# baoxuezhao/GPU-mapreduce

Measured on AMD Instinct MI355X. Metric: KV-pairs/sec (whole node), InvertedIndex end-to-end, higher is better.
Workload: dtype bytes+int32 (no float compute in MapReduce); 1 GPU; model=InvertedIndex, global_batch=1073741824, seq_len=134217728, parallelism=dp1, bytes_per_gpu=1073741824, link_gap=200

## Files before the change

### csrc/engine/engine.cpp

```cpp
#include "hostarena.h"
#include "kv.h"
#include "xfer.h"
#include "grouper.h"

#include <ATen/hip/HIPContext.h>
#include <algorithm>
#include <chrono>
#include <cstring>
#include <condition_variable>
#include <cstdlib>
#include <map>
#include <mutex>
#include <thread>
#include <numeric>
#include <stdexcept>

#include "../kernels/hashfn.h"
#include "../kernels/launch.h"
#include "../kernels/rmatfn.h"

namespace mrh {

namespace {

// ... 1596 lines not shown
  at::Tensor out = at::empty({nval}, opt(dev, at::kLong));
  const int64_t* sp = P0<int64_t>(seg);
  int64_t* o = P0<int64_t>(out);
  int64_t s = 0;
  for (int64_t i = 0; i < nval; ++i) {
    while (s + 1 < nseg && sp[s + 1] <= i) ++s;
    o[i] = s;
  }
  return out;
}

at::Tensor bincount_dev(const at::Tensor& idx_in, int64_t K) {
  const at::Device dev = idx_in.device();
  at::Tensor idx = idx_in.to(at::kLong).contiguous();
  at::Tensor c = at::zeros({std::max<int64_t>(K, 0)}, opt(dev, at::kLong));
  if (idx.numel() == 0 || K <= 0) return c;
  if (dev.is_cuda()) {
    k::histogram(P0<int64_t>(idx), idx.numel(), K, P0<int64_t>(c), cur_stream());
    return c;
  }
  const int64_t* p = P0<int64_t>(idx);
  int64_t* o = P0<int64_t>(c);
  for (int64_t i = 0; i < idx.numel(); ++i)
    if (p[i] >= 0 && p[i] < K) o[p[i]]++;
  return c;
}

at::Tensor mask_indices(const at::Tensor& mask_in) {
  const at::Device dev = mask_in.device();
  at::Tensor m = mask_in.to(at::kBool).contiguous().view(at::kByte);
  const int64_t n = m.numel();
  if (!dev.is_cuda()) return at::nonzero(m).view({-1});
  if (n == 0) return at::empty({0}, opt(dev, at::kLong));
  at::Tensor f = at::empty({n}, opt(dev, at::kLong));
  k::mask_flags(P0<uint8_t>(m), n, P0<int64_t>(f), cur_stream());
  at::Tensor pos = exclusive_scan(f);
  const int64_t cnt = pos[n].item<int64_t>();
  at::Tensor out = at::empty({cnt}, opt(dev, at::kLong));
  if (cnt) k::compact_mask(P0<uint8_t>(m), P0<int64_t>(pos), n, P0<int64_t>(out), cur_stream());
  return out;
}

at::Tensor repeat_index(const at::Tensor& counts) {
  at::Tensor off = exclusive_scan(counts.to(at::kLong));
  const int64_t n = counts.numel();
  const int64_t tot = n ? off[n].item<int64_t>() : 0;
  return segment_ids(off, n, tot);
}

KV expand(const KMV& kmv) {
  at::Tensor sid = segment_ids(kmv.seg, kmv.nkey, kmv.nval);
  KV out;
  out.n = kmv.nval;
  out.kw = kmv.keys.kw;
  out.kdata = gather_rows(kmv.keys.kdata, kmv.keys.koff, kmv.keys.kw, sid, &out.koff);
  out.vw = kmv.vw;
  out.vdata = kmv.vdata;
  out.voff = kmv.voff;
  return out;
}

KMV sort_multivalues(const KMV& kmv, int flag) {
  if (kmv.nval <= 1) return kmv;
  const at::Device dev = kmv.seg.device();
  at::Tensor perm1 = sort_perm_column(kmv.vdata, kmv.voff, kmv.vw, kmv.nval, flag);
  at::Tensor sid = segment_ids(kmv.seg, kmv.nkey, kmv.nval);
  at::Tensor sid_p = sid.index_select(0, perm1.to(at::kLong));
  auto [ks, perm2, passes] = radix_sort_pairs(sid_p, iota_u32(kmv.nval, dev), 0, 64);
  at::Tensor perm = perm1.to(at::kLong).index_select(0, perm2.to(at::kLong));
  KMV out = kmv;
  out.vdata = gather_rows(kmv.vdata, kmv.voff, kmv.vw, perm, &out.voff);
  return out;
}


KV map_urls(const at::Tensor& text, int64_t n, int32_t doc_id) {
  const at::Device dev = text.device();
  if (text.numel() < n + 32) fail("map_urls: text buffer must be padded by >= 32 bytes");
  KV kv;
  kv.kw = -1;
  kv.vw = 4;
  if (dev.is_cuda()) {
    auto s = cur_stream();
    int64_t nt = k::url_num_tiles(n);
    at::Tensor cnt = at::empty({std::max<int64_t>(nt, 1)}, opt(dev, at::kInt));
    k::url_count(P0<uint8_t>(text), n, P0<uint32_t>(cnt), s);
    at::Tensor toff = scan_u32(cnt.narrow(0, 0, nt));
    int64_t nurl = (int64_t)(uint32_t)toff[nt].item<int32_t>();
    at::Tensor starts = at::empty({std::max<int64_t>(nurl, 1)}, opt(dev, at::kLong));
    k::url_emit_starts(P0<uint8_t>(text), n, P0<uint32_t>(toff), P0<int64_t>(starts), s);
    at::Tensor klen = at::empty({std::max<int64_t>(nurl, 1)}, opt(dev, at::kInt));
    k::url_lengths(P0<uint8_t>(text), n, P0<int64_t>(starts), nurl, P0<int32_t>(klen), s);
    kv.koff = exclusive_scan(klen.narrow(0, 0, nurl));
    int64_t kb = scalar_i64(kv.koff, nurl);
    kv.kdata = at::empty({kb}, opt(dev, at::kByte));
    k::url_copy(P0<uint8_t>(text), P0<int64_t>(starts), P0<int64_t>(kv.koff), nurl, P0<uint8_t>(kv.kdata), s);
    at::Tensor v = at::empty({nurl}, opt(dev, at::kInt));
    k::fill_i32(P0<int32_t>(v), nurl, doc_id, s);
    kv.vdata = v.view(at::kByte);
    kv.n = nurl;
    return kv;
  }
  const uint8_t* t = P0<uint8_t>(text);
  static const char pat[] = "<a href=\"";
  std::vector<int64_t> koff{0};
  std::vector<uint8_t> kd;
  for (int64_t i = 0; i + 8 < n; ++i) {
    if (memcmp(t + i, pat, 9) != 0) continue;
    int64_t a = i + 9, j = a;
    while (j < n && t[j] != '"') ++j;
    kd.insert(kd.end(), t + a, t + j);
    kd.push_back(0);
    koff.push_back((int64_t)kd.size());
  }
  kv.n = (int64_t)koff.size() - 1;
  kv.koff = at::from_blob(koff.data(), {(int64_t)koff.size()}, opt(at::kCPU, at::kLong)).clone();
  kv.kdata = at::from_blob(kd.data(), {(int64_t)kd.size()}, opt(at::kCPU, at::kByte)).clone();
  kv.vdata = at::full({kv.n}, doc_id, opt(at::kCPU, at::kInt)).view(at::kByte);
  return kv;
}

static inline bool is_ws(uint8_t c) { return c == ' ' || c == '\t' || c == '\n' || c == '\f' || c == '\r' || c == 0; }

KV map_words(const at::Tensor& text, int64_t n) {
  const at::Device dev = text.device();
  if (text.numel() < n + 32) fail("map_words: text buffer must be padded by >= 32 bytes");
  KV kv;
  kv.kw = -1;
  kv.vw = 0;
  kv.vdata = at::empty({0}, opt(dev, at::kByte));
  if (dev.is_cuda()) {
    auto s = cur_stream();
    const int64_t nt = k::tok_num_tiles(n);
    if (nt <= 0) {
      kv.n = 0;
      kv.koff = at::zeros({1}, opt(dev, at::kLong));
      kv.kdata = at::empty({0}, opt(dev, at::kByte));
      return kv;
    }
    at::Tensor cw = at::empty({nt}, opt(dev, at::kInt)), cb = at::empty({nt}, opt(dev, at::kInt));
    k::tok_count2(P0<uint8_t>(text), n, P0<uint32_t>(cw), P0<uint32_t>(cb), s);
    at::Tensor tw = scan_u32(cw);
    at::Tensor tb = exclusive_scan(cb);
    uint32_t nw32 = 0;
    int64_t kb = 0;
    read_small(s, {{P0<uint32_t>(tw) + nt, &nw32, 4}, {P0<int64_t>(tb) + nt, &kb, 8}});
    const int64_t nw = (int64_t)nw32;
    kv.koff = at::empty({nw + 1}, opt(dev, at::kLong));
    kv.kdata = at::empty({kb}, opt(dev, at::kByte));
    k::tok_emit2(P0<uint8_t>(text), n, P0<uint32_t>(tw), P0<int64_t>(tb), P0<int64_t>(kv.koff), P0<uint8_t>(kv.kdata),
                 s);
    k::fill_i64(P0<int64_t>(kv.koff) + nw, 1, kb, s);
    kv.n = nw;
    return kv;
  }
  const uint8_t* t = P0<uint8_t>(text);
  std::vector<int64_t> koff{0};
  std::vector<uint8_t> kd;
  for (int64_t i = 0; i < n;) {
    while (i < n && is_ws(t[i])) ++i;
    if (i >= n) break;
    int64_t j = i;
    while (j < n && !is_ws(t[j])) ++j;
    kd.insert(kd.end(), t + i, t + j);
    kd.push_back(0);
    koff.push_back((int64_t)kd.size());
    i = j;
  }
  kv.n = (int64_t)koff.size() - 1;
  kv.koff = at::from_blob(koff.data(), {(int64_t)koff.size()}, opt(at::kCPU, at::kLong)).clone();
  kv.kdata = at::from_blob(kd.data(), {(int64_t)kd.size()}, opt(at::kCPU, at::kByte)).clone();
  return kv;
}

KV map_rmat(int64_t nedges, int nlevels, double a, double b, double c, double d, double fraction, uint64_t seed,
            uint64_t first_edge, at::Device dev) {
  KV kv;
  kv.kw = 16;
  kv.vw = 0;
  kv.n = nedges;
  kv.vdata = at::empty({0}, opt(dev, at::kByte));
// ... 16 lines not shown
```

### csrc/kernels/group.hip

```cpp
#include <algorithm>

#include "common.h"
#include "launch.h"

namespace mrh {
namespace k {
namespace {

using dev::rot32;

constexpr int NT = 256;
constexpr int32_t NONE = -1;

unsigned blocks_for(int64_t n) {
  int64_t b = (n + NT - 1) / NT;
  return (unsigned)(b < 1 ? 1 : (b > (1 << 20) ? (1 << 20) : b));
}

__device__ __forceinline__ uint64_t nz(uint64_t h) { return h ? h : 1ull; }
__device__ __forceinline__ uint64_t home(uint64_t h, uint64_t mask) { return (h ^ (h >> 32)) & mask; }

struct Keys {
  const uint8_t* d;
  const int64_t* off;
  int w;
  __device__ __forceinline__ const uint8_t* at(int64_t r) const { return off ? d + off[r] : d + r * (int64_t)w; }
  __device__ __forceinline__ int64_t len(int64_t r) const { return off ? off[r + 1] - off[r] : (int64_t)w; }
};

__device__ __forceinline__ void load_key16(const uint8_t* p, int64_t len, uint32_t w[4]) {
  const uintptr_t a = reinterpret_cast<uintptr_t>(p);
  const uint32_t* q = reinterpret_cast<const uint32_t*>(a & ~uintptr_t(3));
  const uint32_t r = (uint32_t)(a & 3);
  const int nb = len < 16 ? (int)len : 16;
  const int nd = (int)((r + nb + 3) >> 2);
  uint32_t d[5];
#pragma unroll
  for (int j = 0; j < 5; ++j) d[j] = j < nd ? q[j] : 0u;
#pragma unroll
  for (int j = 0; j < 4; ++j) {
    uint32_t v = r ? __builtin_amdgcn_alignbyte(d[j + 1], d[j], r) : d[j];
    const int valid = nb - 4 * j;
    if (valid <= 0) v = 0;
    else if (valid < 4) v &= (1u << (8 * valid)) - 1u;
    w[j] = v;
  }
}

__device__ __forceinline__ uint64_t hash64_words(const uint32_t w[4], int64_t len) {
  uint32_t a, b, c;
  a = b = c = 0xdeadbeefu + (uint32_t)len + 0x9e3779b9u;
  c += 0x7f4a7c15u;
  if (len == 0) return ((uint64_t)c << 32) | b;
  a += w[0];
  b += w[1];
  c += w[2];
  if (len > 12) {
    MRH_L3_MIX(a, b, c);
    a += w[3];
  }
  MRH_L3_FINAL(a, b, c);
  return ((uint64_t)c << 32) | b;
}

__device__ __forceinline__ uint64_t ld_l2_u64(const void* p) {
  return __hip_atomic_load(reinterpret_cast<const unsigned long long*>(p), __ATOMIC_RELAXED,
                           __HIP_MEMORY_SCOPE_AGENT);
}

__global__ __launch_bounds__(NT) void k_dict_insert(Keys K, const uint64_t* __restrict__ h, int64_t n, int64_t row0,
                                                   DictTable T, int32_t* __restrict__ gid, int retry) {
  unsigned long long bad = 0, left = 0;
  const int64_t stride = (int64_t)gridDim.x * NT;
  for (int64_t i = (int64_t)blockIdx.x * NT + threadIdx.x; i - threadIdx.x < n; i += stride) {
    const int64_t row = row0 + i;
    bool live = i < n;
    if (live && retry) live = gid[row] == NONE;
    unsigned long long hv = 0;
    const uint8_t* p = nullptr;
    int64_t len = 0;
    uint32_t w[4] = {0, 0, 0, 0};
    uint64_t s = 0;
    uint4 hdr = make_uint4(0, 0, 0, 0);
    int state = 0;
    if (live) {
      p = K.at(row);
      len = K.len(row);
      load_key16(p, len, w);
      if (h) {
        hv = nz(h[i]);
      } else if (len <= 16) {
        hv = nz(hash64_words(w, len));
      } else {
        uint32_t c = 0x9e3779b9u, b = 0x7f4a7c15u;
        dev::lookup3_wide(p, len, &c, &b);
        hv = nz(((uint64_t)c << 32) | b);
      }
      s = home(hv, T.mask);
      for (uint64_t probe = 0;; ++probe) {
        hdr = *reinterpret_cast<const uint4*>(&T.slots[s]);
        unsigned long long v = ((unsigned long long)hdr.y << 32) | hdr.x;
        if (v == 0) {
          if (__hip_atomic_load(&T.ctr[3], __ATOMIC_RELAXED, __HIP_MEMORY_SCOPE_AGENT)) {
            state = 3;
            break;
          }
          v = atomicCAS(&T.slots[s].hash, 0ull, hv);
          if (v == 0) {
            state = 2;
            break;
          }
          hdr.z = 0;
        }
        if (v == hv) {
          state = 1;
          break;
        }
        s = (s + 1) & T.mask;
        if (probe >= T.mask) {
          state = 3;
          break;
        }
      }
    }
    int32_t g = NONE;
    if (state == 2) {
      g = (int32_t)atomicAdd(&T.ctr[0], 1ull);
      DictSlot& sl = T.slots[s];
      sl.len = (int32_t)len;
      *reinterpret_cast<uint4*>(sl.key) = make_uint4(w[0], w[1], w[2], w[3]);
      T.rep[g] = row;
      T.ghash[g] = hv;
      __hip_atomic_store(&sl.gid1, g + 1, __ATOMIC_RELEASE, __HIP_MEMORY_SCOPE_AGENT);
      if ((int64_t)g + 1 >= T.limit) __hip_atomic_store(&T.ctr[3], 1ull, __ATOMIC_RELAXED, __HIP_MEMORY_SCOPE_AGENT);
    }
    if (state == 1) {
      const DictSlot& sl = T.slots[s];
      bool fresh = false;
      while (hdr.z == 0) {
        __builtin_amdgcn_s_sleep(1);
        const uint64_t gl = ld_l2_u64(&sl.gid1);
        hdr.z = (uint32_t)gl;
        hdr.w = (uint32_t)(gl >> 32);
        fresh = true;
      }
      g = (int32_t)hdr.z - 1;
      uint4 kk = fresh ? make_uint4(0, 0, 0, 0) : *reinterpret_cast<const uint4*>(sl.key);
      bool same = !fresh && (int64_t)(int32_t)hdr.w == len && kk.x == w[0] && kk.y == w[1] && kk.z == w[2] &&
                  kk.w == w[3];
      if (!same) {
        const uint64_t k01 = ld_l2_u64(&sl.key[0]), k23 = ld_l2_u64(&sl.key[2]);
        const uint64_t gl = ld_l2_u64(&sl.gid1);
        same = (int64_t)(int32_t)(gl >> 32) == len && (uint32_t)k01 == w[0] && (uint32_t)(k01 >> 32) == w[1] &&
               (uint32_t)k23 == w[2] && (uint32_t)(k23 >> 32) == w[3];
      }
      if (same && len > 16) {
        int64_t b = T.rep[g];
        if (b < 0) b = (int64_t)ld_l2_u64(&T.rep[g]);
        same = dev::bytes_equal(p + 16, K.at(b) + 16, len - 16);
      }
      if (!same) ++bad;
    }
    if (state == 3) ++left;
    if (live) gid[row] = g;
  }
  bad = dev::wave_sum(bad);
  left = dev::wave_sum(left);
  if (dev::lane_id() == 0) {
    if (bad) atomicAdd(&T.ctr[1], bad);
    if (left) atomicAdd(&T.ctr[2], left);
  }
}

constexpr int HW = 32768;
constexpr int HNT = 1024;
constexpr int kDictHistRows = 256;

__global__ __launch_bounds__(HNT) void k_dict_hist(const int32_t* __restrict__ gid, int64_t n, int64_t w0,
                                                  int64_t wlen, uint32_t* __restrict__ partial) {
  __shared__ uint32_t hist[HW];
  for (int j = threadIdx.x; j < HW; j += HNT) hist[j] = 0;
  __syncthreads();
  const int64_t n4 = n >> 2;
  const int4* g4 = reinterpret_cast<const int4*>(gid);
  auto add = [&](int32_t g) {
    const uint64_t d = (uint64_t)((int64_t)g - w0);
// ... 178 lines not shown
```

### csrc/kernels/launch.h

```cpp
#pragma once
#include <hip/hip_runtime.h>
#include <cstddef>
#include <cstdint>

namespace mrh {
namespace k {

size_t scan_temp_bytes(int64_t n);
void exclusive_scan_u32(const uint32_t* in, uint32_t* out, int64_t n, void* temp, hipStream_t s);
void exclusive_scan_i64(const int64_t* in, int64_t* out, int64_t n, void* temp, hipStream_t s);
void lengths_to_offsets(const int32_t* len, int64_t* off, int64_t n, void* temp, hipStream_t s);

size_t radix_temp_bytes(int64_t n);
void radix_sort_u64_u32(const uint64_t* keys_in, const uint32_t* vals_in, uint64_t* keys_out,
                        uint32_t* vals_out, uint64_t* keys_alt, uint32_t* vals_alt, int64_t n,
                        int begin_bit, int end_bit, void* temp, hipStream_t s,
                        int* passes_run = nullptr, bool skip_trivial = true);

void hash32_fixed(const uint8_t* kdata, int kw, int64_t n, uint32_t seed, uint32_t* out, hipStream_t s);
void hash32_var(const uint8_t* kdata, const int64_t* koff, int64_t n, uint32_t seed, uint32_t* out,
                hipStream_t s);
void hash64_fixed(const uint8_t* kdata, int kw, int64_t n, uint64_t* out, hipStream_t s);
void hash64_var(const uint8_t* kdata, const int64_t* koff, int64_t n, uint64_t* out, hipStream_t s);
void partition_dest(const uint32_t* h, int64_t n, int P, int32_t* dest, int64_t* counts, hipStream_t s);

int part_tile();
void part_count(const int32_t* dest_in, const uint8_t* kd, int kw, const int64_t* koff, const int64_t* voff,
                int64_t n, int P, int nb, int32_t* dest_out, int64_t* cnt, int64_t* kbytes, int64_t* vbytes,
                hipStream_t s);
void part_scatter(const int32_t* dest, int64_t n, int P, int nb, const int64_t* cbase, const uint8_t* kd, int kw,
                  const uint8_t* vd, int vw, const int64_t* koff, const int64_t* voff, uint8_t* ksend,
                  uint8_t* vsend, int64_t* perm, int32_t* klen, int32_t* vlen, hipStream_t s);
void copy_var_i64(const uint8_t* src, const int64_t* soff, const int64_t* perm, int64_t n, uint8_t* dst,
                  const int64_t* doff, hipStream_t s);
void part_header(const int64_t* cs, const int64_t* ks, const int64_t* vs, int P, int nb, int kw, int vw,
                 int64_t kcode, int64_t vcode, int64_t* hdr, hipStream_t s);
void count_mod(const int64_t* v, int64_t n, int P, int64_t* counts, hipStream_t s);
void piece_bytes(const int64_t* soff, const int64_t* start, int P, int R, int64_t* out, hipStream_t s);

void seg_marks(const int64_t* seg, int64_t nseg, int64_t nval, int64_t* marks, hipStream_t s);
void histogram(const int64_t* idx, int64_t n, int64_t K, int64_t* counts, hipStream_t s);
void nz_flags(const uint64_t* v, int64_t n, int32_t* f, hipStream_t s);
void compact_nz(const uint64_t* v, const int64_t* pos, int64_t n, int64_t* out, hipStream_t s);
void mask_flags(const uint8_t* m, int64_t n, int64_t* f, hipStream_t s);
void compact_mask(const uint8_t* m, const int64_t* pos, int64_t n, int64_t* out, hipStream_t s);
void lookup_sorted(const int64_t* keys, int64_t n, const int64_t* q, int64_t m, int64_t* idx, hipStream_t s);

void make_sortkeys_fixed(const uint8_t* data, int w, int64_t n, int mode, bool descending,
                         uint64_t* keys, uint32_t* idx, hipStream_t s);
void make_sortkeys_strprefix(const uint8_t* data, const int64_t* off, int64_t n, int64_t start,
                             bool descending, uint64_t* keys, uint32_t* idx, hipStream_t s);
void iota_u32(uint32_t* idx, int64_t n, hipStream_t s);
void str_groups(const uint64_t* ks, const uint8_t* alive, const uint32_t* head_in, int64_t n, bool desc,
                uint32_t* head_out, hipStream_t s);
void str_active(const uint64_t* ks, const uint8_t* alive, const uint32_t* head, int64_t n, bool desc, uint32_t* active,
                hipStream_t s);
void str_refine(const uint32_t* active, const uint32_t* pos, const uint32_t* gid_incl, const uint32_t* perm,
                const uint8_t* data, const int64_t* off, int64_t n, int64_t start, bool desc, int32_t* where,
                uint64_t* nk, uint64_t* gk, hipStream_t s);
void str_apply(const uint32_t* order, const int32_t* where, const uint64_t* nk, int64_t m, const uint32_t* perm_in,
               uint32_t* perm_out, uint64_t* ks, uint8_t* alive, hipStream_t s);
void gather_fixed(const uint8_t* src, int w, const uint32_t* idx, int64_t n, uint8_t* dst, hipStream_t s);
void gather_fixed_i64idx(const uint8_t* src, int w, const int64_t* idx, int64_t n, uint8_t* dst,
                         hipStream_t s);
void gather_var_lengths(const int64_t* src_off, const uint32_t* idx, int64_t n, int32_t* len,
                        hipStream_t s);
void gather_var_copy(const uint8_t* src, const int64_t* src_off, const uint32_t* idx, int64_t n,
                     uint8_t* dst, const int64_t* dst_off, hipStream_t s);
void head_flags_u64(const uint64_t* keys, int64_t n, uint32_t* flags, hipStream_t s);
void compact_heads(const uint32_t* flags, const uint32_t* pos, int64_t n, int64_t* seg, hipStream_t s);
struct PackShifts {
  int nw;
  int s[8];
};
void pack_words(const uint64_t* kd, int64_t n, const PackShifts& sh, uint64_t* out, uint32_t* idx, hipStream_t s);
void pack_kv(const uint64_t* kd, const uint64_t* vd, int64_t n, const PackShifts& sh, uint64_t* out, hipStream_t s);
void pack_kv_split(const uint64_t* kd, const void* vd, int vw, int64_t n, const PackShifts& sh, int vbits, int B, int hi,
                   uint64_t* out, int32_t* bkt, hipStream_t s);
void unpack_split(const uint64_t* heads, int64_t m, int bucket, int B, int hi, const PackShifts& sh,
                  const PackShifts& bits, uint64_t* keys, hipStream_t s);
void split_values(const uint64_t* words, int64_t n, int vbits, int vw, void* vout, hipStream_t s);
int64_t seg_packed_tiles(int64_t n);
void seg_packed_count(const uint64_t* w, int64_t n, int vb, uint64_t km, int64_t* tcnt, hipStream_t s);
void seg_packed_write(const uint64_t* w, int64_t n, int vb, uint64_t km, const int64_t* tbase, int64_t* seg,
                      uint64_t* heads, void* vout, int vw, hipStream_t s);
void bits_count(const uint64_t* H, int64_t nw, uint32_t* cnt, hipStream_t s);
void bits_compact(const uint64_t* H, int64_t nw, const uint32_t* pos, int64_t n, int64_t* seg, hipStream_t s);
void verify_groups_var(const uint8_t* kdata, const int64_t* koff, const uint32_t* perm,
                       const uint32_t* flags, const uint32_t* pos, const int64_t* seg, int64_t n,
                       unsigned long long* mismatches, hipStream_t s);
void verify_groups_fixed(const uint8_t* kdata, int kw, const uint32_t* perm, const uint32_t* flags,
                         const uint32_t* pos, const int64_t* seg, int64_t n,
                         unsigned long long* mismatches, hipStream_t s);
void dest_byte_counts(const int32_t* dest, const int64_t* off, int64_t n, int P, int64_t* bytes,
                      hipStream_t s);
void offsets_to_lengths(const int64_t* off, int64_t n, int32_t* len, hipStream_t s);

void seg_reduce(const void* vals, int dtype, int op, const int64_t* seg, int64_t nseg, int64_t nval, void* out,
                hipStream_t s);
void seg_count(const int64_t* seg, int64_t nseg, int32_t* out, hipStream_t s);

int64_t url_num_tiles(int64_t n);
void url_count(const uint8_t* text, int64_t n, uint32_t* tile_counts, hipStream_t s);
void url_emit_starts(const uint8_t* text, int64_t n, const uint32_t* tile_off, int64_t* starts,
                     hipStream_t s);
void url_lengths(const uint8_t* text, int64_t n, const int64_t* starts, int64_t nurl,
                 int32_t* keylen, hipStream_t s);
void url_copy(const uint8_t* text, const int64_t* starts, const int64_t* koff, int64_t nurl,
              uint8_t* kdata, hipStream_t s);
int64_t tok_num_tiles(int64_t n);
void tok_count2(const uint8_t* text, int64_t n, uint32_t* tile_words, uint32_t* tile_bytes, hipStream_t s);
void tok_emit2(const uint8_t* text, int64_t n, const uint32_t* toff_w, const int64_t* toff_b, int64_t* koff,
               uint8_t* kd, hipStream_t s);
void tok_count(const uint8_t* text, int64_t n, uint32_t* tile_counts, hipStream_t s);
void tok_emit(const uint8_t* text, int64_t n, const uint32_t* tile_off, int64_t* starts,
              int32_t* keylen, hipStream_t s);
void copy_strings_nul(const uint8_t* text, const int64_t* starts, const int64_t* koff, int64_t n,
                      uint8_t* kdata, hipStream_t s);
void fill_i32(int32_t* p, int64_t n, int32_t v, hipStream_t s);
void bucket_by_splitters(const uint64_t* keys, int64_t n, const uint64_t* split, int nsplit, int32_t* out,
                         hipStream_t s, bool right = false);

void rmat_edges(uint64_t* edges, int64_t nedges, int nlevels, float a, float b, float c, float d,
                float fraction, uint64_t seed, uint64_t first_edge, hipStream_t s);

size_t pr_scratch_bytes(int64_t nval);
void pr_contrib(const int64_t* seg, int64_t nseg, int64_t nedge, const int32_t* src, const float* w, const float* r,
                float* out, void* scratch, hipStream_t s);
void pr_combine(const int64_t* seg, int64_t ngrp, int64_t nrecv, const int32_t* perm, const float* recv,
                const int32_t* vid, float* grp, float* acc, void* scratch, hipStream_t s);
void scatter_f32(const float* v, const int32_t* idx, int64_t n, float* out, hipStream_t s);
int pr_update_blocks(int64_t n);
void pr_pack_src(const int64_t* e, int64_t n, int P, bool swap, uint64_t* out, hipStream_t s);
void pr_heads(const uint64_t* sorted, int64_t n, uint32_t* flags, hipStream_t s);
void pr_run_degree(const uint64_t* sorted, const int64_t* seg, int64_t nrun, uint32_t* deg, hipStream_t s);
void pr_degkey(const uint32_t* deg, int64_t n, uint64_t* key, uint32_t* iota, hipStream_t s);
void pr_relabel(const uint32_t* order, const uint32_t* deg, int64_t n, int32_t* nid, int64_t* order64,
                uint8_t* dangling, float* invdeg, unsigned long long* ndangling, int32_t* degn, hipStream_t s);
void sample_i64(const int64_t* in, int64_t n, int64_t stride, int64_t ns, int64_t* out, hipStream_t s);
void pr_pack(const uint64_t* su, int64_t n, int P, int64_t nlmax, bool local, bool swapped, const int32_t* nid,
             const int32_t* rb, int nr, int dbits, uint64_t* out, hipStream_t s);
void pr_mix_pack(const int64_t* e, int64_t n, int P, int64_t N, bool mix, uint64_t* out, int32_t* dest, hipStream_t s);
void pr_localize(uint64_t* p, int64_t n, int P, hipStream_t s);
void pr_pack_dst(const uint64_t* su, int64_t n, int P, int64_t base, const int32_t* nid, uint64_t* out, int32_t* dest,
                 hipStream_t s);
void pr_pack_gather(const uint64_t* in, int64_t n, int P, int64_t S, const int32_t* nid, const int32_t* rb, int nr,
                    int dbits, uint64_t* out, hipStream_t s);
void pr_unmix_ids(const int64_t* order, int64_t n, int P, int me, int64_t N, bool mix, int64_t* ids, hipStream_t s);
void pr_unpack(const uint64_t* sorted, int64_t n, int32_t* src, uint32_t* flags, hipStream_t s);
void pr_deg_window(const uint64_t* e, int64_t m, int shift, uint32_t* deg, hipStream_t s);
void pr_unpack_bits(const uint64_t* sorted, int64_t n, int32_t* src, uint32_t* H, hipStream_t s);
void pr_group_hi(const uint64_t* sorted, const int64_t* seg, int64_t ngrp, int64_t* hi, hipStream_t s);
void pr_group_vid(const int64_t* hi, int64_t ngrp, const int32_t* nid, int64_t dmask, int32_t* vid, hipStream_t s);
int pr_tile_bits();
void pr_range_offsets(const int64_t* hi, int64_t ngrp, int dbits, int R, int64_t ntile, int64_t* off, hipStream_t s);
void pr_partials_sum(const double* part, int64_t ntile, double* stats, hipStream_t s);
void pr_tile_step(const float* send, const int32_t* ghi, const int64_t* off, int R, int64_t ntile, int64_t ndst,
                  const float* r, float* rn, const uint8_t* dangling, float base, float alpha, const double* dmass,
                  double invN, const float* invdeg, float* cout, double* partial, hipStream_t s);
void pr_update(float* acc, const float* r, float* rn, const uint8_t* dangling, int64_t n, float base,
               float alpha, const double* dmass, double invN, const float* invdeg, float* cout, double* partial,
               hipStream_t s);

size_t plan_scratch_bytes(int64_t n);
void plan_gather_reduce(int dtype, const int64_t* seg, int64_t nseg, int64_t ne, const int32_t* src, const void* x,
                        const void* w, int op, void* out, void* scratch, hipStream_t s);
void plan_combine(int dtype, const int64_t* seg, int64_t ngrp, int64_t nrecv, const int32_t* perm, const void* recv,
                  const int32_t* vid, int op, void* grp, void* acc, void* scratch, hipStream_t s);
int64_t ws_words(int64_t nval);
int64_t ws_waves(int64_t nval);
void ws_index(const int64_t* seg, int64_t nseg, int64_t nval, uint32_t* H, int64_t* wbase, hipStream_t s);
void ws_bases(const int64_t* seg, int64_t nseg, int64_t nval, int64_t* wbase, hipStream_t s);
size_t ws_scratch_bytes(int64_t nval);
void ws_gather_reduce(int dtype, const uint32_t* H, const int64_t* wbase, int64_t nval, const int32_t* src,
                      const void* x, const void* w, int op, void* out, void* scratch, hipStream_t s,
                      const int32_t* sched = nullptr, int64_t slen = 0, int64_t nx = 0);
int64_t wedge_tiles(int64_t nwedge);
void wedges(const int64_t* seg, const int64_t* gidx, const int64_t* wscan, int64_t ngw, const int64_t* nb,
            const int64_t* centre, int64_t w0, int64_t nwedge, int64_t* out_edge, int64_t* out_centre, int64_t* tg,
            hipStream_t s);
void wedges_compact(const int64_t* seg, const int64_t* gidx, const int64_t* wscan, int64_t ngw, const int64_t* nb,
                    const int64_t* centre, int64_t w0, int64_t nwedge, int vb, int64_t* out_key, uint32_t* out_centre,
                    int64_t* tg, hipStream_t s);

int pb_bin_size();
void pb_phase1(const int32_t* src, const int32_t* out_pos, int64_t m, const float* c, float* vals, hipStream_t s);
void pb_phase2(const float* vals, const uint16_t* dst, const int32_t* ub, const int64_t* ue0, const int64_t* ue1,
               const uint8_t* uex, int64_t nunit, int64_t nv, float* acc, hipStream_t s);
void pb_layout(const int32_t* perm2, const int32_t* dst1, int64_t m, int32_t* out_pos, uint16_t* dst2, hipStream_t s);

void tri_pack(const int64_t* e, int64_t n, int64_t nvert, uint64_t* out, unsigned int* bad, hipStream_t s);
void tri_col(const uint64_t* okeys, int64_t m, uint32_t* col, hipStream_t s);
// ... 178 lines not shown
```

### csrc/kernels/text.hip

```cpp
#include "common.h"
#include "launch.h"
#include <cstdio>
#include <cstdlib>

namespace mrh {
namespace k {
namespace {

constexpr int NT = 256;
constexpr int BYTES_PER_THREAD = 16;
constexpr int TILE = NT * BYTES_PER_THREAD;

constexpr uint32_t P0 = 0x6820613Cu;
constexpr uint32_t P1 = 0x3D666572u;
constexpr uint32_t P2 = 0x22u;

__device__ __forceinline__ uint32_t align_bytes(uint32_t hi, uint32_t lo, int r) {
  return __builtin_amdgcn_alignbyte(hi, lo, (uint32_t)r);
}

__device__ __forceinline__ void load_window(const uint8_t* text, int64_t p, uint32_t w[8]) {
  uint4 a = *reinterpret_cast<const uint4*>(text + p);
  uint2 b = *reinterpret_cast<const uint2*>(text + p + 16);
  uint32_t c = *reinterpret_cast<const uint32_t*>(text + p + 24);
  w[0] = a.x; w[1] = a.y; w[2] = a.z; w[3] = a.w; w[4] = b.x; w[5] = b.y; w[6] = c; w[7] = 0;
}

__device__ __forceinline__ uint32_t url_match_mask(const uint8_t* text, int64_t p, int64_t n) {
  uint32_t w[8];
  load_window(text, p, w);
  uint32_t m = 0;
#pragma unroll
  for (int k = 0; k < BYTES_PER_THREAD; ++k) {
    const int q = k >> 2, r = k & 3;
    uint32_t x0 = r ? align_bytes(w[q + 1], w[q], r) : w[q];
    uint32_t x1 = r ? align_bytes(w[q + 2], w[q + 1], r) : w[q + 1];
    uint32_t x2 = (r ? align_bytes(w[q + 3], w[q + 2], r) : w[q + 2]) & 0xffu;
    bool hit = (x0 == P0) & (x1 == P1) & (x2 == P2) & (p + k + 8 < n);
    m |= (uint32_t)hit << k;
  }
  return m;
}

__global__ __launch_bounds__(NT) void k_url_count(const uint8_t* __restrict__ text, int64_t n,
                                                 uint32_t* __restrict__ tile_counts) {
  __shared__ uint32_t sh[NT / MRH_WAVE];
  const int64_t p = (int64_t)blockIdx.x * TILE + (int64_t)threadIdx.x * BYTES_PER_THREAD;
  uint32_t c = (p < n) ? (uint32_t)__popc(url_match_mask(text, p, n)) : 0u;
  c = dev::wave_sum(c);
  if (dev::lane_id() == 0) sh[dev::wave_id()] = c;
  __syncthreads();
  if (threadIdx.x == 0) tile_counts[blockIdx.x] = sh[0] + sh[1] + sh[2] + sh[3];
}

__global__ __launch_bounds__(NT) void k_url_emit(const uint8_t* __restrict__ text, int64_t n,
                                                const uint32_t* __restrict__ tile_off,
                                                int64_t* __restrict__ starts) {
  __shared__ uint32_t sh[NT / MRH_WAVE + 1];
  const int64_t p = (int64_t)blockIdx.x * TILE + (int64_t)threadIdx.x * BYTES_PER_THREAD;
  uint32_t m = (p < n) ? url_match_mask(text, p, n) : 0u;
  uint32_t total;
  uint32_t pos = dev::block_excl_scan<uint32_t, NT>((uint32_t)__popc(m), sh, &total);
  int64_t o = (int64_t)tile_off[blockIdx.x] + pos;
  while (m) {
    int k = __ffs(m) - 1;
    m &= m - 1;
    starts[o++] = p + k + 9;
  }
}

__global__ __launch_bounds__(NT) void k_url_len(const uint8_t* __restrict__ text, int64_t n,
                                               const int64_t* __restrict__ starts, int64_t nurl,
                                               int32_t* __restrict__ keylen) {
  int64_t i = (int64_t)blockIdx.x * NT + threadIdx.x;
  if (i >= nurl) return;
  int64_t a = starts[i];
  int64_t len = dev::find_byte(text + a, n - a, (uint8_t)'"');
  keylen[i] = (int32_t)(len + 1);
}

__device__ __forceinline__ bool is_ws(uint32_t c) {
  return c == ' ' || c == '\t' || c == '\n' || c == '\f' || c == '\r' || c == 0;
}

__device__ __forceinline__ uint32_t word_start_mask(const uint8_t* text, int64_t p, int64_t n) {
  uint4 a = *reinterpret_cast<const uint4*>(text + p);
  uint32_t prev = (p == 0) ? 0u : (uint32_t)text[p - 1];
  uint32_t w[4] = {a.x, a.y, a.z, a.w};
  uint32_t m = 0;
  bool prev_ws = is_ws(prev);
#pragma unroll
  for (int k = 0; k < 16; ++k) {
    uint32_t c = (w[k >> 2] >> (8 * (k & 3))) & 0xffu;
    bool ws = is_ws(c) | (p + k >= n);
    m |= (uint32_t)(!ws && prev_ws) << k;
    prev_ws = ws;
  }
  return m;
}

__global__ __launch_bounds__(NT) void k_tok_count(const uint8_t* __restrict__ text, int64_t n,
                                                 uint32_t* __restrict__ tile_counts) {
  __shared__ uint32_t sh[NT / MRH_WAVE];
  const int64_t p = (int64_t)blockIdx.x * TILE + (int64_t)threadIdx.x * 16;
  uint32_t c = (p < n) ? (uint32_t)__popc(word_start_mask(text, p, n)) : 0u;
  c = dev::wave_sum(c);
  if (dev::lane_id() == 0) sh[dev::wave_id()] = c;
  __syncthreads();
  if (threadIdx.x == 0) tile_counts[blockIdx.x] = sh[0] + sh[1] + sh[2] + sh[3];
}

__global__ __launch_bounds__(NT) void k_tok_emit(const uint8_t* __restrict__ text, int64_t n,
                                                const uint32_t* __restrict__ tile_off,
                                                int64_t* __restrict__ starts, int32_t* __restrict__ keylen) {
  __shared__ uint32_t sh[NT / MRH_WAVE + 1];
  const int64_t p = (int64_t)blockIdx.x * TILE + (int64_t)threadIdx.x * 16;
  uint32_t m = (p < n) ? word_start_mask(text, p, n) : 0u;
  uint32_t total;
  uint32_t pos = dev::block_excl_scan<uint32_t, NT>((uint32_t)__popc(m), sh, &total);
  int64_t o = (int64_t)tile_off[blockIdx.x] + pos;
  while (m) {
    int k = __ffs(m) - 1;
    m &= m - 1;
    int64_t a = p + k, j = a;
    while (j < n && !is_ws(text[j])) ++j;
    starts[o] = a;
    keylen[o] = (int32_t)(j - a + 1);
    ++o;
  }
}

__device__ __forceinline__ void word_masks(const uint8_t* text, int64_t p, int64_t n, uint32_t* S, uint32_t* E,
                                           uint32_t* B) {
  const uint4 a = *reinterpret_cast<const uint4*>(text + p);
  const uint32_t nxt = (uint32_t)text[p + 16];
  const uint32_t prev = (p == 0) ? 0u : (uint32_t)text[p - 1];
  const uint32_t w[4] = {a.x, a.y, a.z, a.w};
  bool ws[18];
  ws[0] = is_ws(prev);
#pragma unroll
  for (int k = 0; k < 16; ++k) ws[k + 1] = is_ws((w[k >> 2] >> (8 * (k & 3))) & 0xffu) | (p + k >= n);
  ws[17] = is_ws(nxt) | (p + 16 >= n);
  uint32_t s = 0, e = 0, b = 0;
#pragma unroll
  for (int k = 0; k < 16; ++k) {
    s |= (uint32_t)(!ws[k + 1] && ws[k]) << k;
    e |= (uint32_t)(!ws[k + 1] && ws[k + 2]) << k;
    b |= (uint32_t)(!ws[k + 1]) << k;
  }
  *S = s;
  *E = e;
  *B = b;
}

__global__ __launch_bounds__(NT) void k_tok_count2(const uint8_t* __restrict__ text, int64_t n,
                                                  uint32_t* __restrict__ tile_words,
                                                  uint32_t* __restrict__ tile_bytes) {
  __shared__ uint32_t sh[2][NT / MRH_WAVE];
  const int64_t p = (int64_t)blockIdx.x * TILE + (int64_t)threadIdx.x * 16;
  uint32_t cw = 0, cb = 0;
  if (p < n) {
// ... 4 lines not shown
  }
  cw = dev::wave_sum(cw);
  cb = dev::wave_sum(cb);
  if (dev::lane_id() == 0) {
    sh[0][dev::wave_id()] = cw;
    sh[1][dev::wave_id()] = cb;
  }
  __syncthreads();
  if (threadIdx.x == 0) {
    tile_words[blockIdx.x] = sh[0][0] + sh[0][1] + sh[0][2] + sh[0][3];
    tile_bytes[blockIdx.x] = sh[1][0] + sh[1][1] + sh[1][2] + sh[1][3];
  }
}

__global__ __launch_bounds__(NT) void k_tok_emit2(const uint8_t* __restrict__ text, int64_t n,
                                                 const uint32_t* __restrict__ toff_w,
                                                 const int64_t* __restrict__ toff_b,
                                                 int64_t* __restrict__ koff, uint8_t* __restrict__ kd) {
  __shared__ uint32_t shw[NT / MRH_WAVE + 1];
  __shared__ uint32_t shb[NT / MRH_WAVE + 1];
  __shared__ __attribute__((aligned(16))) uint8_t sbytes[2 * TILE + 16];
  __shared__ int64_t soffs[TILE / 2 + 1];
  const int64_t p = (int64_t)blockIdx.x * TILE + (int64_t)threadIdx.x * 16;
  uint32_t S = 0, E = 0, B = 0;
  if (p < n) word_masks(text, p, n, &S, &E, &B);
  uint32_t tw, tb;
  const uint32_t pw = dev::block_excl_scan<uint32_t, NT>((uint32_t)__popc(S), shw, &tw);
  const uint32_t pb = dev::block_excl_scan<uint32_t, NT>((uint32_t)(__popc(B) + __popc(E)), shb, &tb);
  const int64_t wb = (int64_t)toff_w[blockIdx.x];
  const int64_t ob = toff_b[blockIdx.x];
  const int lead = (int)((reinterpret_cast<uintptr_t>(kd) + (uintptr_t)ob) & 15);
  if (S | B) {
    uint32_t w = pw, o = pb;
    const uint4 a = *reinterpret_cast<const uint4*>(text + p);
    const uint32_t wd[4] = {a.x, a.y, a.z, a.w};
#pragma unroll
    for (int k = 0; k < 16; ++k) {
      if ((S >> k) & 1u) soffs[w++] = ob + o;
      if ((B >> k) & 1u) sbytes[lead + o++] = (uint8_t)((wd[k >> 2] >> (8 * (k & 3))) & 0xffu);
      if ((E >> k) & 1u) sbytes[lead + o++] = 0;
    }
  }
  __syncthreads();
  for (uint32_t i = threadIdx.x; i < tw; i += NT) koff[wb + i] = soffs[i];
  const int64_t base = ob - lead, end = ob + tb;
  const int64_t nchunk = (end - base + 15) >> 4;
  for (int64_t c = threadIdx.x; c < nchunk; c += NT) {
    const int64_t g0 = base + 16 * c;
    if (g0 >= ob && g0 + 16 <= end) {
      *reinterpret_cast<uint4*>(kd + g0) = *reinterpret_cast<const uint4*>(sbytes + 16 * c);
    } else {
      for (int k = 0; k < 16; ++k) {
        const int64_t g = g0 + k;
        if (g >= ob && g < end) kd[g] = sbytes[16 * c + k];
      }
    }
  }
}

__global__ __launch_bounds__(NT) void k_copy_nul(const uint8_t* __restrict__ text,
                                                const int64_t* __restrict__ starts,
                                                const int64_t* __restrict__ koff, int64_t n,
                                                uint8_t* __restrict__ kd) {
  const int g = threadIdx.x & 15;
  int64_t row = ((int64_t)blockIdx.x * NT + threadIdx.x) >> 4;
  const int64_t stride = ((int64_t)gridDim.x * NT) >> 4;
  for (; row < n; row += stride) {
    int64_t a = starts[row], o = koff[row], len = koff[row + 1] - o - 1;
    for (int64_t j = g; j < len; j += 16) kd[o + j] = text[a + j];
    if (g == 0) kd[o + len] = 0;
  }
}

__global__ __launch_bounds__(NT) void k_fill_i32(int32_t* p, int64_t n, int32_t v) {
  int64_t i = (int64_t)blockIdx.x * NT + threadIdx.x;
  if (i < n) p[i] = v;
}

}

int64_t url_num_tiles(int64_t n) { return (n + TILE - 1) / TILE; }
int64_t tok_num_tiles(int64_t n) { return (n + TILE - 1) / TILE; }

void url_count(const uint8_t* text, int64_t n, uint32_t* tile_counts, hipStream_t s) {
  int64_t nt = url_num_tiles(n);
  if (nt <= 0) return;
  hipLaunchKernelGGL(k_url_count, dim3((unsigned)nt), dim3(NT), 0, s, text, n, tile_counts);
  MRH_CHECK_LAUNCH();
}
void url_emit_starts(const uint8_t* text, int64_t n, const uint32_t* tile_off, int64_t* starts,
                     hipStream_t s) {
  int64_t nt = url_num_tiles(n);
  if (nt <= 0) return;
  hipLaunchKernelGGL(k_url_emit, dim3((unsigned)nt), dim3(NT), 0, s, text, n, tile_off, starts);
  MRH_CHECK_LAUNCH();
}
void url_lengths(const uint8_t* text, int64_t n, const int64_t* starts, int64_t nurl, int32_t* keylen,
                 hipStream_t s) {
  if (nurl <= 0) return;
  hipLaunchKernelGGL(k_url_len, dim3((unsigned)((nurl + NT - 1) / NT)), dim3(NT), 0, s, text, n, starts,
                     nurl, keylen);
  MRH_CHECK_LAUNCH();
}
void copy_strings_nul(const uint8_t* text, const int64_t* starts, const int64_t* koff, int64_t n,
                      uint8_t* kdata, hipStream_t s) {
  if (n <= 0) return;
  int64_t g = (n * 16 + NT - 1) / NT;
  if (g > 65536) g = 65536;
  hipLaunchKernelGGL(k_copy_nul, dim3((unsigned)g), dim3(NT), 0, s, text, starts, koff, n, kdata);
  MRH_CHECK_LAUNCH();
}
void url_copy(const uint8_t* text, const int64_t* starts, const int64_t* koff, int64_t nurl,
              uint8_t* kdata, hipStream_t s) {
  copy_strings_nul(text, starts, koff, nurl, kdata, s);
}
void tok_count2(const uint8_t* text, int64_t n, uint32_t* tile_words, uint32_t* tile_bytes, hipStream_t s) {
  const int64_t nt = tok_num_tiles(n);
  if (nt <= 0) return;
  hipLaunchKernelGGL(k_tok_count2, dim3((unsigned)nt), dim3(NT), 0, s, text, n, tile_words, tile_bytes);
  MRH_CHECK_LAUNCH();
}
void tok_emit2(const uint8_t* text, int64_t n, const uint32_t* toff_w, const int64_t* toff_b, int64_t* koff,
               uint8_t* kd, hipStream_t s) {
  const int64_t nt = tok_num_tiles(n);
  if (nt <= 0) return;
  hipLaunchKernelGGL(k_tok_emit2, dim3((unsigned)nt), dim3(NT), 0, s, text, n, toff_w, toff_b, koff, kd);
  MRH_CHECK_LAUNCH();
}
void tok_count(const uint8_t* text, int64_t n, uint32_t* tile_counts, hipStream_t s) {
  int64_t nt = tok_num_tiles(n);
  if (nt <= 0) return;
  hipLaunchKernelGGL(k_tok_count, dim3((unsigned)nt), dim3(NT), 0, s, text, n, tile_counts);
  MRH_CHECK_LAUNCH();
}
void tok_emit(const uint8_t* text, int64_t n, const uint32_t* tile_off, int64_t* starts, int32_t* keylen,
              hipStream_t s) {
  int64_t nt = tok_num_tiles(n);
  if (nt <= 0) return;
  hipLaunchKernelGGL(k_tok_emit, dim3((unsigned)nt), dim3(NT), 0, s, text, n, tile_off, starts, keylen);
  MRH_CHECK_LAUNCH();
}
void fill_i32(int32_t* p, int64_t n, int32_t v, hipStream_t s) {
  if (n <= 0) return;
  hipLaunchKernelGGL(k_fill_i32, dim3((unsigned)((n + NT - 1) / NT)), dim3(NT), 0, s, p, n, v);
  MRH_CHECK_LAUNCH();
}

}
}
```

Before: 280.9 million KV/s.

## Fuse URL map into two-pass count/emit kernels with shared-memory staged output

Replaces the four-kernel URL extraction (count, emit starts, lengths, copy) plus fill and scan with two kernels. The count pass computes per-tile URL counts and byte totals using per-thread quote masks in shared memory. The emit pass writes offsets, values and key bytes directly, staging output in LDS for aligned vector stores. This removes intermediate start/length arrays, extra launches and one host sync. It also hoists the table-full atomic load out of the probe loop in dict insert, which may delay detecting a full table until retry.

```diff
diff --git a/csrc/engine/engine.cpp b/csrc/engine/engine.cpp
--- a/csrc/engine/engine.cpp
+++ b/csrc/engine/engine.cpp
@@ -1702,21 +1702,27 @@
   kv.vw = 4;
   if (dev.is_cuda()) {
     auto s = cur_stream();
-    int64_t nt = k::url_num_tiles(n);
-    at::Tensor cnt = at::empty({std::max<int64_t>(nt, 1)}, opt(dev, at::kInt));
-    k::url_count(P0<uint8_t>(text), n, P0<uint32_t>(cnt), s);
-    at::Tensor toff = scan_u32(cnt.narrow(0, 0, nt));
-    int64_t nurl = (int64_t)(uint32_t)toff[nt].item<int32_t>();
-    at::Tensor starts = at::empty({std::max<int64_t>(nurl, 1)}, opt(dev, at::kLong));
-    k::url_emit_starts(P0<uint8_t>(text), n, P0<uint32_t>(toff), P0<int64_t>(starts), s);
-    at::Tensor klen = at::empty({std::max<int64_t>(nurl, 1)}, opt(dev, at::kInt));
-    k::url_lengths(P0<uint8_t>(text), n, P0<int64_t>(starts), nurl, P0<int32_t>(klen), s);
-    kv.koff = exclusive_scan(klen.narrow(0, 0, nurl));
-    int64_t kb = scalar_i64(kv.koff, nurl);
+    const int64_t nt = k::url_num_tiles(n);
+    if (nt <= 0) {
+      kv.n = 0;
+      kv.koff = at::zeros({1}, opt(dev, at::kLong));
+      kv.kdata = at::empty({0}, opt(dev, at::kByte));
+      kv.vdata = at::empty({0}, opt(dev, at::kByte));
+      return kv;
+    }
+    at::Tensor cu = at::empty({nt}, opt(dev, at::kInt)), cb = at::empty({nt}, opt(dev, at::kLong));
+    k::url_count2(P0<uint8_t>(text), n, P0<uint32_t>(cu), P0<int64_t>(cb), s);
+    at::Tensor tu = scan_u32(cu);
+    at::Tensor tb = exclusive_scan(cb);
+    uint32_t nurl32 = 0;
+    int64_t kb = 0;
+    read_small(s, {{P0<uint32_t>(tu) + nt, &nurl32, 4}, {P0<int64_t>(tb) + nt, &kb, 8}});
+    const int64_t nurl = (int64_t)nurl32;
+    kv.koff = at::empty({nurl + 1}, opt(dev, at::kLong));
     kv.kdata = at::empty({kb}, opt(dev, at::kByte));
-    k::url_copy(P0<uint8_t>(text), P0<int64_t>(starts), P0<int64_t>(kv.koff), nurl, P0<uint8_t>(kv.kdata), s);
     at::Tensor v = at::empty({nurl}, opt(dev, at::kInt));
-    k::fill_i32(P0<int32_t>(v), nurl, doc_id, s);
+    k::url_emit2(P0<uint8_t>(text), n, P0<uint32_t>(tu), P0<int64_t>(tb), doc_id, P0<int64_t>(kv.koff),
+                 P0<uint8_t>(kv.kdata), P0<int32_t>(v), s);
     kv.vdata = v.view(at::kByte);
     kv.n = nurl;
     return kv;
diff --git a/csrc/kernels/group.hip b/csrc/kernels/group.hip
--- a/csrc/kernels/group.hip
+++ b/csrc/kernels/group.hip
@@ -83,6 +83,7 @@
     uint64_t s = 0;
     uint4 hdr = make_uint4(0, 0, 0, 0);
     int state = 0;
+    const bool full = __hip_atomic_load(&T.ctr[3], __ATOMIC_RELAXED, __HIP_MEMORY_SCOPE_AGENT) != 0;
     if (live) {
       p = K.at(row);
       len = K.len(row);
@@ -101,7 +102,7 @@
         hdr = *reinterpret_cast<const uint4*>(&T.slots[s]);
         unsigned long long v = ((unsigned long long)hdr.y << 32) | hdr.x;
         if (v == 0) {
-          if (__hip_atomic_load(&T.ctr[3], __ATOMIC_RELAXED, __HIP_MEMORY_SCOPE_AGENT)) {
+          if (full) {
             state = 3;
             break;
           }
diff --git a/csrc/kernels/launch.h b/csrc/kernels/launch.h
--- a/csrc/kernels/launch.h
+++ b/csrc/kernels/launch.h
@@ -101,13 +101,9 @@
 void seg_count(const int64_t* seg, int64_t nseg, int32_t* out, hipStream_t s);
 
 int64_t url_num_tiles(int64_t n);
-void url_count(const uint8_t* text, int64_t n, uint32_t* tile_counts, hipStream_t s);
-void url_emit_starts(const uint8_t* text, int64_t n, const uint32_t* tile_off, int64_t* starts,
-                     hipStream_t s);
-void url_lengths(const uint8_t* text, int64_t n, const int64_t* starts, int64_t nurl,
-                 int32_t* keylen, hipStream_t s);
-void url_copy(const uint8_t* text, const int64_t* starts, const int64_t* koff, int64_t nurl,
-              uint8_t* kdata, hipStream_t s);
+void url_count2(const uint8_t* text, int64_t n, uint32_t* tile_urls, int64_t* tile_bytes, hipStream_t s);
+void url_emit2(const uint8_t* text, int64_t n, const uint32_t* toff_u, const int64_t* toff_b, int32_t doc_id,
+               int64_t* koff, uint8_t* kd, int32_t* vd, hipStream_t s);
 int64_t tok_num_tiles(int64_t n);
 void tok_count2(const uint8_t* text, int64_t n, uint32_t* tile_words, uint32_t* tile_bytes, hipStream_t s);
 void tok_emit2(const uint8_t* text, int64_t n, const uint32_t* toff_w, const int64_t* toff_b, int64_t* koff,
diff --git a/csrc/kernels/text.hip b/csrc/kernels/text.hip
--- a/csrc/kernels/text.hip
+++ b/csrc/kernels/text.hip
@@ -26,57 +26,154 @@
   w[0] = a.x; w[1] = a.y; w[2] = a.z; w[3] = a.w; w[4] = b.x; w[5] = b.y; w[6] = c; w[7] = 0;
 }
 
-__device__ __forceinline__ uint32_t url_match_mask(const uint8_t* text, int64_t p, int64_t n) {
+__device__ __forceinline__ void url_masks(const uint8_t* text, int64_t p, int64_t n, uint32_t* M, uint32_t* Q) {
   uint32_t w[8];
   load_window(text, p, w);
-  uint32_t m = 0;
+  uint32_t m = 0, q = 0;
 #pragma unroll
   for (int k = 0; k < BYTES_PER_THREAD; ++k) {
-    const int q = k >> 2, r = k & 3;
-    uint32_t x0 = r ? align_bytes(w[q + 1], w[q], r) : w[q];
-    uint32_t x1 = r ? align_bytes(w[q + 2], w[q + 1], r) : w[q + 1];
-    uint32_t x2 = (r ? align_bytes(w[q + 3], w[q + 2], r) : w[q + 2]) & 0xffu;
+    const int i = k >> 2, r = k & 3;
+    uint32_t x0 = r ? align_bytes(w[i + 1], w[i], r) : w[i];
+    uint32_t x1 = r ? align_bytes(w[i + 2], w[i + 1], r) : w[i + 1];
+    uint32_t x2 = (r ? align_bytes(w[i + 3], w[i + 2], r) : w[i + 2]) & 0xffu;
     bool hit = (x0 == P0) & (x1 == P1) & (x2 == P2) & (p + k + 8 < n);
     m |= (uint32_t)hit << k;
-  }
-  return m;
-}
-
-__global__ __launch_bounds__(NT) void k_url_count(const uint8_t* __restrict__ text, int64_t n,
-                                                 uint32_t* __restrict__ tile_counts) {
-  __shared__ uint32_t sh[NT / MRH_WAVE];
-  const int64_t p = (int64_t)blockIdx.x * TILE + (int64_t)threadIdx.x * BYTES_PER_THREAD;
-  uint32_t c = (p < n) ? (uint32_t)__popc(url_match_mask(text, p, n)) : 0u;
+    q |= (uint32_t)(((x0 & 0xffu) == P2) & (p + k < n)) << k;
+  }
+  *M = m;
+  *Q = q;
+}
+
+__device__ __forceinline__ int64_t url_len(const uint8_t* text, int64_t n, int64_t t0, const uint16_t* sq,
+                                           int64_t a) {
+  const int64_t r = a - t0;
+  int t = (int)(r >> 4);
+  if (t < NT) {
+    const uint32_t mk = (uint32_t)sq[t] >> (r & 15);
+    if (mk) return __ffs(mk) - 1;
+    for (++t; t < NT; ++t) {
+      const uint32_t q = sq[t];
+      if (q) return (int64_t)t * 16 + (__ffs(q) - 1) - r;
+    }
+  }
+  const int64_t pos = a > t0 + TILE ? a : t0 + TILE;
+  if (pos >= n) return n - a;
+  return pos - a + dev::find_byte(text + pos, n - pos, (uint8_t)'"');
+}
+
+__global__ __launch_bounds__(NT) void k_url_count2(const uint8_t* __restrict__ text, int64_t n,
+                                                  uint32_t* __restrict__ tile_urls,
+                                                  int64_t* __restrict__ tile_bytes) {
+  __shared__ uint16_t sq[NT];
+  __shared__ uint32_t shc[NT / MRH_WAVE];
+  __shared__ unsigned long long shb[NT / MRH_WAVE];
+  const int64_t t0 = (int64_t)blockIdx.x * TILE;
+  const int64_t p = t0 + (int64_t)threadIdx.x * BYTES_PER_THREAD;
+  uint32_t M = 0, Q = 0;
+  if (p < n) url_masks(text, p, n, &M, &Q);
+  sq[threadIdx.x] = (uint16_t)Q;
+  __syncthreads();
+  uint32_t c = (uint32_t)__popc(M);
+  unsigned long long b = 0;
+  while (M) {
+    const int k = __ffs(M) - 1;
+    M &= M - 1;
+    b += (unsigned long long)url_len(text, n, t0, sq, p + k + 9) + 1ull;
+  }
   c = dev::wave_sum(c);
-  if (dev::lane_id() == 0) sh[dev::wave_id()] = c;
-  __syncthreads();
-  if (threadIdx.x == 0) tile_counts[blockIdx.x] = sh[0] + sh[1] + sh[2] + sh[3];
-}
-
-__global__ __launch_bounds__(NT) void k_url_emit(const uint8_t* __restrict__ text, int64_t n,
-                                                const uint32_t* __restrict__ tile_off,
-                                                int64_t* __restrict__ starts) {
-  __shared__ uint32_t sh[NT / MRH_WAVE + 1];
-  const int64_t p = (int64_t)blockIdx.x * TILE + (int64_t)threadIdx.x * BYTES_PER_THREAD;
-  uint32_t m = (p < n) ? url_match_mask(text, p, n) : 0u;
-  uint32_t total;
-  uint32_t pos = dev::block_excl_scan<uint32_t, NT>((uint32_t)__popc(m), sh, &total);
-  int64_t o = (int64_t)tile_off[blockIdx.x] + pos;
-  while (m) {
-    int k = __ffs(m) - 1;
-    m &= m - 1;
-    starts[o++] = p + k + 9;
-  }
-}
-
-__global__ __launch_bounds__(NT) void k_url_len(const uint8_t* __restrict__ text, int64_t n,
-                                               const int64_t* __restrict__ starts, int64_t nurl,
-                                               int32_t* __restrict__ keylen) {
-  int64_t i = (int64_t)blockIdx.x * NT + threadIdx.x;
-  if (i >= nurl) return;
-  int64_t a = starts[i];
-  int64_t len = dev::find_byte(text + a, n - a, (uint8_t)'"');
-  keylen[i] = (int32_t)(len + 1);
+  b = dev::wave_sum(b);
+  if (dev::lane_id() == 0) {
+    shc[dev::wave_id()] = c;
+    shb[dev::wave_id()] = b;
+  }
+  __syncthreads();
+  if (threadIdx.x == 0) {
+    tile_urls[blockIdx.x] = shc[0] + shc[1] + shc[2] + shc[3];
+    tile_bytes[blockIdx.x] = (int64_t)(shb[0] + shb[1] + shb[2] + shb[3]);
+  }
+}
+
+constexpr int URLS_PER_TILE = (TILE + 8) / 9;
+
+__global__ __launch_bounds__(NT) void k_url_emit2(const uint8_t* __restrict__ text, int64_t n,
+                                                 const uint32_t* __restrict__ toff_u,
+                                                 const int64_t* __restrict__ toff_b, int32_t doc_id,
+                                                 int64_t* __restrict__ koff, uint8_t* __restrict__ kd,
+                                                 int32_t* __restrict__ vd) {
+  __shared__ uint16_t sq[NT];
+  __shared__ uint32_t shu[NT / MRH_WAVE + 1];
+  __shared__ unsigned long long shb[NT / MRH_WAVE + 1];
+  __shared__ __attribute__((aligned(16))) uint8_t sbytes[TILE + 32];
+  __shared__ int64_t slen[URLS_PER_TILE];
+  __shared__ uint32_t ssrc[URLS_PER_TILE];
+  __shared__ uint32_t sout[URLS_PER_TILE];
+  const int64_t t0 = (int64_t)blockIdx.x * TILE;
+  const int64_t p = t0 + (int64_t)threadIdx.x * BYTES_PER_THREAD;
+  uint32_t M = 0, Q = 0;
+  if (p < n) url_masks(text, p, n, &M, &Q);
+  sq[threadIdx.x] = (uint16_t)Q;
+  __syncthreads();
+  int64_t len[2] = {0, 0};
+  uint32_t src[2] = {0, 0};
+  int cnt = 0;
+  unsigned long long b = 0;
+  while (M && cnt < 2) {
+    const int k = __ffs(M) - 1;
+    M &= M - 1;
+    const int64_t a = p + k + 9;
+    src[cnt] = (uint32_t)(a - t0);
+    len[cnt] = url_len(text, n, t0, sq, a);
+    b += (unsigned long long)len[cnt] + 1ull;
+    ++cnt;
+  }
+  uint32_t tu;
+  unsigned long long tb;
+  const uint32_t pu = dev::block_excl_scan<uint32_t, NT>((uint32_t)cnt, shu, &tu);
+  const unsigned long long pb = dev::block_excl_scan<unsigned long long, NT>(b, shb, &tb);
+  const int64_t ub = (int64_t)toff_u[blockIdx.x];
+  const int64_t ob = toff_b[blockIdx.x];
+  const int lead = (int)((reinterpret_cast<uintptr_t>(kd) + (uintptr_t)ob) & 15);
+  if (cnt > 0) {
+    ssrc[pu] = src[0];
+    sout[pu] = (uint32_t)pb;
+    slen[pu] = len[0];
+  }
+  if (cnt > 1) {
+    ssrc[pu + 1] = src[1];
+    sout[pu + 1] = (uint32_t)(pb + (unsigned long long)len[0] + 1ull);
+    slen[pu + 1] = len[1];
+  }
+  __syncthreads();
+  const int g = threadIdx.x & 15;
+  for (uint32_t u = threadIdx.x >> 4; u < tu; u += NT / 16) {
+    const uint8_t* s = text + t0 + ssrc[u];
+    const int64_t o = (int64_t)sout[u], l = slen[u];
+    for (int64_t j = g; j <= l; j += 16) {
+      const uint8_t c = j < l ? s[j] : (uint8_t)0;
+      const int64_t d = o + j;
+      if (d < TILE) sbytes[lead + d] = c;
+      else kd[ob + d] = c;
+    }
+  }
+  __syncthreads();
+  for (uint32_t i = threadIdx.x; i < tu; i += NT) {
+    koff[ub + i] = ob + (int64_t)sout[i];
+    vd[ub + i] = doc_id;
+  }
+  if (blockIdx.x == gridDim.x - 1 && threadIdx.x == 0) koff[ub + tu] = ob + (int64_t)tb;
+  const int64_t base = ob - lead, end = ob + (int64_t)(tb < (unsigned long long)TILE ? tb : (unsigned long long)TILE);
+  const int64_t nchunk = (end - base + 15) >> 4;
+  for (int64_t c = threadIdx.x; c < nchunk; c += NT) {
+    const int64_t g0 = base + 16 * c;
+    if (g0 >= ob && g0 + 16 <= end) {
+      *reinterpret_cast<uint4*>(kd + g0) = *reinterpret_cast<const uint4*>(sbytes + 16 * c);
+    } else {
+      for (int k = 0; k < 16; ++k) {
+        const int64_t gb = g0 + k;
+        if (gb >= ob && gb < end) kd[gb] = sbytes[16 * c + k];
+      }
+    }
+  }
 }
 
 __device__ __forceinline__ bool is_ws(uint32_t c) {
@@ -247,24 +344,17 @@
 int64_t url_num_tiles(int64_t n) { return (n + TILE - 1) / TILE; }
 int64_t tok_num_tiles(int64_t n) { return (n + TILE - 1) / TILE; }
 
-void url_count(const uint8_t* text, int64_t n, uint32_t* tile_counts, hipStream_t s) {
-  int64_t nt = url_num_tiles(n);
-  if (nt <= 0) return;
-  hipLaunchKernelGGL(k_url_count, dim3((unsigned)nt), dim3(NT), 0, s, text, n, tile_counts);
-  MRH_CHECK_LAUNCH();
-}
-void url_emit_starts(const uint8_t* text, int64_t n, const uint32_t* tile_off, int64_t* starts,
-                     hipStream_t s) {
-  int64_t nt = url_num_tiles(n);
-  if (nt <= 0) return;
-  hipLaunchKernelGGL(k_url_emit, dim3((unsigned)nt), dim3(NT), 0, s, text, n, tile_off, starts);
-  MRH_CHECK_LAUNCH();
-}
-void url_lengths(const uint8_t* text, int64_t n, const int64_t* starts, int64_t nurl, int32_t* keylen,
-                 hipStream_t s) {
-  if (nurl <= 0) return;
-  hipLaunchKernelGGL(k_url_len, dim3((unsigned)((nurl + NT - 1) / NT)), dim3(NT), 0, s, text, n, starts,
-                     nurl, keylen);
+void url_count2(const uint8_t* text, int64_t n, uint32_t* tile_urls, int64_t* tile_bytes, hipStream_t s) {
+  const int64_t nt = url_num_tiles(n);
+  if (nt <= 0) return;
+  hipLaunchKernelGGL(k_url_count2, dim3((unsigned)nt), dim3(NT), 0, s, text, n, tile_urls, tile_bytes);
+  MRH_CHECK_LAUNCH();
+}
+void url_emit2(const uint8_t* text, int64_t n, const uint32_t* toff_u, const int64_t* toff_b, int32_t doc_id,
+               int64_t* koff, uint8_t* kd, int32_t* vd, hipStream_t s) {
+  const int64_t nt = url_num_tiles(n);
+  if (nt <= 0) return;
+  hipLaunchKernelGGL(k_url_emit2, dim3((unsigned)nt), dim3(NT), 0, s, text, n, toff_u, toff_b, doc_id, koff, kd, vd);
   MRH_CHECK_LAUNCH();
 }
 void copy_strings_nul(const uint8_t* text, const int64_t* starts, const int64_t* koff, int64_t n,
@@ -275,10 +365,6 @@
   hipLaunchKernelGGL(k_copy_nul, dim3((unsigned)g), dim3(NT), 0, s, text, starts, koff, n, kdata);
   MRH_CHECK_LAUNCH();
 }
-void url_copy(const uint8_t* text, const int64_t* starts, const int64_t* koff, int64_t nurl,
-              uint8_t* kdata, hipStream_t s) {
-  copy_strings_nul(text, starts, koff, nurl, kdata, s);
-}
 void tok_count2(const uint8_t* text, int64_t n, uint32_t* tile_words, uint32_t* tile_bytes, hipStream_t s) {
   const int64_t nt = tok_num_tiles(n);
   if (nt <= 0) return;
```

After: 281.3 million KV/s (median of 3 runs). About the same (+0.2%).
